# Isaac-McPadden/Farkle_II

Measured on AMD Instinct MI355X. Metric: simulated games/sec (whole node) at k=2, fixed strategy-grid size, higher is better.
Workload: dtype int32; 1 GPU; BASELINE configs[1]: k=2, 64-strategy grid, 10^7 games per GPU per step, root_seed 42, counts-only tallies; k=2, root_seed=42, parallelism=shuffle-range split x1, device=AMD Radeon Graphics, arch=gfx950:sramecc+:xnack-, compute_units=256, clock_mhz=2400

## Files before the change

### farkle_ii_amd/csrc/farkle_hip.hip

```cpp
#include "fk_kernels.h"
#include "fk_shard_writer.h"
#include "fk_perm_wave.h"
#include "fk_row_columns_seats.h"
#include "fk_matchups.h"
#include "fk_game_stats.h"
#include "fk_bootstrap.h"
#include "fk_root_stability.h"

#include <dlfcn.h>
#include <rccl/rccl.h>
#include <unistd.h>

#include <algorithm>
#include <atomic>
#include <chrono>
#include <cmath>
#include <memory>
#include <mutex>
#include <sys/mman.h>
#include <unordered_map>
#include <thread>
#include <cstdarg>
#include <cstdio>
#include <cstring>
// ... 51 lines not shown
    int32_t hint_state = 0, pipeline = 1;
    hipDeviceProp_t prop{};
    std::string err;
    fk_timing timing{};
    std::string play_instance;
    hipEvent_t ev[8] = {nullptr, nullptr, nullptr, nullptr, nullptr, nullptr, nullptr, nullptr};
    int32_t *err_host = nullptr;
    hipEvent_t main_idle = nullptr;
    struct PendingTimer {
        float *acc;
        hipEvent_t a, b;
    };
    std::vector<PendingTimer> pending;
    DevBuf strat, recs, rec0, tally, rows, ov, seatlist, coords, inv, slow, score_lut, discard_lut, block_out, stats, ratios, digest,
        dbg[6];
    std::vector<uint2> strat_host;
    int32_t longest_first = 1;
    int32_t blocks_per_cu = 0;
    int32_t max_waves = 6;
    int32_t lean = -1;
    int32_t gs = -1;
    int32_t uniform_flags_opt = -1;
    uint32_t table_flags = 0;
    uint32_t table_mixed_flags = 0xff00u;
    int64_t chunk_bytes = (int64_t)48 << 30;
    int32_t workspace_percent = 80;
    int64_t chunk_limit = 0;
    int64_t last_budget = 0;
    bool oom = false;
    std::vector<void *> hog;
    int32_t oom_replays = 0;
    int32_t batch_threshold = 0;
    int32_t use_lds_tally = -1;
    int32_t block = 0;
    int32_t hc = -1;
    int32_t hc_waves = 5;
    int32_t hc_block = 256;
    int32_t hc_tables = 1;
    int32_t hc_inc_regs = 1;
    int32_t hc_cl = -1;
    DevBuf lds_tables;
    DevBuf cold;
    int32_t clock_stamps = 0;
    DevBuf clk;
    int clk_grid = 0;
    DevBuf lag_v, lag_out, lag_lags, lag_edge, lag_tmp;
    DevBuf m_ids, m_dig, m_seat, m_rnd;
    DevBuf mr[36];
    uint64_t matchup_sort_mask = ~0ull;
    DevBuf g_rec, g_out;
    int64_t game_stats_window = 0;
    const GameStatsReq *gstats = nullptr;
    DevBuf rootb[4];
    DevBuf boot[8];
    int64_t bootstrap_block = 0;
    bool ran_hc = false;
    int32_t perm_split = -1;
    int32_t columns_by_seat = -1;
    int32_t perm_draw_wave = -1;
    void *comm = nullptr;
    int comm_rank = 0, comm_world = 1;
    bool comm_async = false;
    bool comm_lost = false;
    bool comm_timeout_set = false;
    int32_t comm_timeout_ms = 120000;
    DevBuf comm_buf;
// ... 146 lines not shown
    for (int64_t i = 0; i < S; ++i)
        if (s[i].consider_dice && (s[i].require_both || !s[i].consider_score))
            patience[(size_t)i] = s[i].dice_threshold < 1 ? 3 : s[i].dice_threshold == 1 ? 2 : s[i].dice_threshold == 2 ? 1 : 0;
    rc = ensure(c, c->slow, patience.size());
    if (rc) return rc;
    HIPCHK(c, hipMemcpyAsync(c->slow.p, patience.data(), patience.size(), hipMemcpyHostToDevice, c->stream));
    HIPCHK(c, hipStreamSynchronize(c->stream));
    c->strat_host.swap(packed);
    return FK_OK;
}

SeedPool seed_prefix(uint32_t purpose, uint64_t root_seed, uint64_t k) {
    SeedPool p;
    ss_begin(p, 2u , purpose, (uint32_t)root_seed, (uint32_t)(root_seed >> 32));
    ss_absorb64(p, k);
    return p;
}

struct LaunchPlan {
    int block = 0, grid = 0, cus = 1;
    mutable int launched_grid = 0;
    mutable const char *instance = nullptr;
    size_t lds = 0;
    bool lds_tally = false;
    bool lean = false;
    bool gs = false;
    bool blk = false;
    bool hc = false;
    bool hc_lt = false;
    int hc_ki = 0;
    bool hc_cl = false;
    int wpe = 4;
    uint32_t mixed_flags = 0xff00u;
};

constexpr size_t LDS_LIMIT = 160 * 1024;

size_t play_lds_bytes(int32_t k, int block, bool lean, bool gs, bool lds_tally, int32_t S, bool blocks_mode = false) {
    const size_t per_lane = (size_t)(lean ? LEAN_DW : NF) * 4 * (size_t)(gs ? 1 : k) + (blocks_mode ? 4 : 0);
    return per_lane * (size_t)block + (lds_tally ? (size_t)S * LT_COLS * 8 : 0);
}

LaunchPlan plan_play(const fk_ctx *c, int32_t k, int64_t S, bool single_batch, int32_t target_score, bool blocks_mode = false) {
    LaunchPlan best;
    const bool lean_ok = ceil_div50(target_score) <= LEAN_MAX_TARGET50;
    if (blocks_mode) {
        if (!lean_ok) return best;
        best.block = 768;
        best.lean = true;
        best.blk = true;
        best.wpe = 6;
        best.lds = play_lds_bytes(2, 768, true, false, false, 0, true);
        const int per_cu = c->blocks_per_cu > 0 ? std::min(2, c->blocks_per_cu) : 2;
        best.grid = c->prop.multiProcessorCount * per_cu;
        best.cus = c->prop.multiProcessorCount;
        return best;
    }
    const bool want_tally = single_batch && !blocks_mode && (c->use_lds_tally != 0) && S <= 4096;
    int best_lanes = -1;
    const bool gs_wanted = c->gs == 1;
    for (int gs = 0; gs <= 1; ++gs) {
        if (gs != (gs_wanted ? 1 : 0) && best_lanes >= 0) continue;
        for (int lean = 0; lean <= 1; ++lean) {
            if (gs && !lean) continue;
            if (lean && !lean_ok) continue;
            if (!gs && c->lean >= 0 && lean != c->lean) continue;
// ... 184 lines not shown
hipError_t launch_play_hc(const LaunchPlan &p, const PlayArgs &a, hipStream_t s) {
    if (p.hc_cl) {
        if (p.block == 320 && a.k <= 4u) return launch_play_hc_t<320, false, 0, 6, false, true, 4>(p, a, s);
        return hipErrorInvalidValue;
    }
    if (p.hc_ki == 3) {
        if (p.block != 768) return hipErrorInvalidValue;
        if (a.k <= 10u) return launch_play_hc_t<768, true, 10, 3, false, false, 10>(p, a, s);
        return launch_play_hc_t<768, true, 12, 3, false, false, 12>(p, a, s);
    }
    if (p.hc_ki == 2) {
        if (a.k == 5u && p.block == 256) return launch_play_hc_t<256, true, 5, 4, false, false, 6>(p, a, s);
        if (a.k == 6u && p.block == 512) return launch_play_hc_t<512, true, 6, 4, false, false, 6>(p, a, s);
        if (a.k == 7u && p.block == 1024) return launch_play_hc_t<1024, true, 7, 4, false>(p, a, s);
        return hipErrorInvalidValue;
    }
    if (p.hc_ki && p.block == 256 && p.hc_lt) {
        if (a.k == 8u) return launch_play_hc_t<256, true, 8>(p, a, s);
    }
    return hipErrorInvalidValue;
}

hipError_t launch_play(const LaunchPlan &p, const PlayArgs &a, hipStream_t s) {
    if (p.lds > LDS_LIMIT) return hipErrorInvalidValue;
    if (p.hc) return launch_play_hc(p, a, s);
    if (p.blk) return launch_play_t<768, true, 6, false, true, 2>(p, a, s);
    if (p.gs) {
        if (p.block == 768) return launch_play_t<768, true, 6, true>(p, a, s);
        return hipErrorInvalidValue;
    }
    if (p.lean) {
        switch (p.block) {
        case 1024: return launch_play_t<1024, true>(p, a, s);
        case 768: return a.k == 2u ? launch_play_t<768, true, 6, false, false, 2>(p, a, s) : launch_play_t<768, true, 6>(p, a, s);
        case 512: return launch_play_t<512, true>(p, a, s);
        case 256: return launch_play_t<256, true>(p, a, s);
        case 128: return launch_play_t<128, true>(p, a, s);
        default: return launch_play_t<64, true>(p, a, s);
        }
    }
    switch (p.block) {
    case 1024: return launch_play_t<1024, false>(p, a, s);
    case 512: return launch_play_t<512, false>(p, a, s);
    case 256: return launch_play_t<256, false>(p, a, s);
    case 128: return launch_play_t<128, false>(p, a, s);
    default: return launch_play_t<64, false>(p, a, s);
    }
}

enum TimerSlot : int { SLOT_PERM = 0, SLOT_SEED = 2, SLOT_PLAY = 4, SLOT_CALL = 6 };

struct Timer {
    fk_ctx *c;
    float *acc;
    hipEvent_t a, b;
    Timer(fk_ctx *ctx, float *dst, int slot) : c(ctx), acc(dst), a(ctx->ev[slot]), b(ctx->ev[slot + 1]) {
        (void)hipEventRecord(a, c->stream);
    }
    void stop() {
        (void)hipEventRecord(b, c->stream);
        c->pending.push_back({acc, a, b});
    }
};

hipError_t collect_timers(fk_ctx *c) {
    hipError_t first = hipSuccess;
    for (const auto &t : c->pending) {
// ... 137 lines not shown
                           sa.blocks ? sa.game_row : nullptr, static_cast<uint32_t *>(cs.classes.p));
    hipLaunchKernelGGL(fk_seed_kernel, dim3((sa.n_games + SEED_BLOCK - 1u) / SEED_BLOCK), dim3(SEED_BLOCK), 0, st, sa);
    if (timed) (void)hipEventRecord(cs.ev[3], st);
    HIPCHK(c, hipGetLastError());
    return FK_OK;
}

size_t game_workspace_bytes(int32_t k, bool full_state, bool recs, bool rows) {
    return (size_t)k * ((full_state ? STATE_DW * 4 : 18) + 16) + 8 + (recs ? REC_DW * 4 + 4 : 0) +
           (rows ? sizeof(fk_row_hdr) + sizeof(fk_seat) * (size_t)k : 0);
}

int launch_play_stage(fk_ctx *c, const SeedArgs &sa, PlayArgs &pa, const LaunchPlan &plan, bool want_state, bool want_rec0, bool want_recs) {
    ChunkSet &cs = CSET(c);
    int rc;
    if (want_rec0) {
        rc = ensure(c, c->rec0, (size_t)sa.n_games * 4);
        if (rc) return rc;
    }
    if (want_recs) {
        rc = ensure(c, c->recs, (size_t)sa.n_games * REC_DW * 4);
        if (rc) return rc;
    }
    pa.sched = sa.sched;
    pa.seat_idx = sa.seat_idx;
    pa.state = sa.state;
    pa.state_dw = sa.state_dw;
    pa.inc = sa.inc;
    pa.rec0 = want_rec0 ? static_cast<uint32_t *>(c->rec0.p) : nullptr;
    pa.recs = want_recs ? static_cast<uint32_t *>(c->recs.p) : nullptr;
    pa.gs_out = (want_state && !plan.gs) ? 1u : 0u;
    pa.ticket = static_cast<uint32_t *>(cs.misc.p);
    pa.err = reinterpret_cast<int32_t *>(static_cast<uint8_t *>(cs.misc.p) + 16);
    const int auto_thr = sa.k >= 11 ? 16 : sa.k >= 9 ? 12 : 8;
    pa.batch_threshold = (uint32_t)std::max(1, std::min(64, c->batch_threshold > 0 ? c->batch_threshold : auto_thr));
    pa.use_lds_tally = plan.lds_tally ? 1u : 0u;
    pa.clk = nullptr;
    c->clk_grid = 0;
    if (c->clock_stamps) {
        const size_t bytes = (size_t)std::max(plan.grid, 1) * 4 * sizeof(unsigned long long);
        rc = ensure(c, c->clk, bytes);
        if (rc) return rc;
        HIPCHK(c, hipMemsetAsync(c->clk.p, 0, bytes, c->stream));
        pa.clk = static_cast<unsigned long long *>(c->clk.p);
    }
    {
        Timer t(c, &c->timing.play_ms, SLOT_PLAY);
        LaunchPlan lp = plan;
        lp.mixed_flags = (c->uniform_flags_opt != 0) ? c->table_mixed_flags : 0xff00u;
        pa.uflags = c->table_flags;
        hipError_t e = launch_play(lp, pa, c->stream);
        t.stop();
        HIPCHK(c, e);
        c->play_instance = lp.instance ? lp.instance : "";
        c->timing.play_grid = lp.launched_grid;
        c->timing.play_mixed_flags = lp.mixed_flags == MIXED_NONE ? (int32_t)MIXED_NONE
                                     : (lp.mixed_flags & ~MIXED_RB_FAV) == 0u ? (int32_t)MIXED_RB_FAV : (int32_t)MIXED_ALL;
        if (pa.clk) c->clk_grid = lp.launched_grid;
    }
    c->timing.play_launches += 1;
    c->timing.play_block = plan.block;
    c->timing.play_lds_bytes = (int32_t)plan.lds;
    c->timing.games += sa.n_games;
    return FK_OK;
}

int finish_timers(fk_ctx *c) {
    HIPCHK(c, collect_timers(c));
    if (c->clk_grid > 0) {
        std::vector<unsigned long long> h((size_t)c->clk_grid * 4);
        HIPCHK(c, hipMemcpy(h.data(), c->clk.p, h.size() * sizeof(unsigned long long), hipMemcpyDeviceToHost));
        std::vector<double> mhz, ends;
        unsigned long long first = ~0ull;
        for (int b = 0; b < c->clk_grid; ++b) {
            const unsigned long long t0 = h[(size_t)b * 4], r0 = h[(size_t)b * 4 + 1], t1 = h[(size_t)b * 4 + 2], r1 = h[(size_t)b * 4 + 3];
            if (r1 > r0 && t1 > t0) {
                mhz.push_back(100.0 * (double)(t1 - t0) / (double)(r1 - r0));
                ends.push_back((double)r1);
                first = r0 < first ? r0 : first;
            }
        }
// ... 493 lines not shown
    if (free_now) *free_now = (int64_t)free_b;
    if (total) *total = (int64_t)total_b;
    return FK_OK;
}

static int32_t effective_comm_timeout_ms(const fk_ctx *c);

int fk_get_option(fk_ctx *c, const char *name, int64_t *value) {
    if (!c || !name || !value) return FK_ERR_ARG;
    const std::string n(name);
    if (n == "chunk_bytes") *value = c->chunk_bytes;
    else if (n == "workspace_percent") *value = c->workspace_percent;
    else if (n == "last_budget") *value = c->last_budget;
    else if (n == "oom_replays") *value = c->oom_replays;
    else if (n == "comm_timeout_ms") *value = effective_comm_timeout_ms(c);
    else if (n == "rows_chunk_games") *value = c->rows_chunk_games;
    else if (n == "rows_async") *value = c->rows_async;
    else if (n == "rows_event") *value = c->last_rows_event;
    else return fail(c, FK_ERR_ARG, "fk_get_option: unknown option %s", name);
    return FK_OK;
}

int fk_set_option(fk_ctx *c, const char *name, int64_t value) {
    if (!c || !name) return FK_ERR_ARG;
    std::string n(name);
    if (n == "chunk_bytes") c->chunk_bytes = std::max<int64_t>(value, 1 << 20);
    else if (n == "workspace_percent") c->workspace_percent = (int32_t)std::min<int64_t>(std::max<int64_t>(value, 1), 100000);
    else if (n == "comm_timeout_ms") {
        c->comm_timeout_ms = (int32_t)std::min<int64_t>(std::max<int64_t>(value, 0), 86400000);
        c->comm_timeout_set = true;
    }
    else if (n == "batch_threshold") c->batch_threshold = (int32_t)value;
    else if (n == "use_lds_tally") c->use_lds_tally = (int32_t)value;
    else if (n == "longest_first") c->longest_first = (int32_t)value;
    else if (n == "blocks_per_cu") c->blocks_per_cu = (int32_t)value;
    else if (n == "max_waves") c->max_waves = (int32_t)std::min<int64_t>(std::max<int64_t>(value, 1), 8);
    else if (n == "lean") c->lean = (int32_t)value;
    else if (n == "state_store") c->gs = (int32_t)value;
    else if (n == "rows_chunk_games") c->rows_chunk_games = std::max<int64_t>(value, 1);
    else if (n == "rows_async") c->rows_async = value != 0;
    else if (n == "resident_tally") {
        c->resident = value != 0;
        c->acc_n = 0;
    } else if (n == "hot_cold") {
        if (value != -1 && value != 0) return fail(c, FK_ERR_ARG, "hot_cold is -1 (auto: four and more seats) or 0 (never)");
        c->hc = (int32_t)value;
    }
    else if (n == "clock_stamps") c->clock_stamps = value != 0;
    else if (n == "perm_split") c->perm_split = (int32_t)value;
    else if (n == "perm_draw_wave") c->perm_draw_wave = (int32_t)value;
    else if (n == "columns_by_seat") c->columns_by_seat = (int32_t)value;
    else if (n == "pipeline") c->pipeline = (int32_t)value;
    else if (n == "uniform_flags") c->uniform_flags_opt = (int32_t)value;
    else if (n == "matchup_sort_key_mask") c->matchup_sort_mask = (uint64_t)value;
    else if (n == "game_stats_window") c->game_stats_window = std::max<int64_t>(value, 0);
    else if (n == "bootstrap_block") c->bootstrap_block = std::max<int64_t>(value, 0);
    else if (n == "block") {
        if (value != 0 && value != 64 && value != 128 && value != 256 && value != 512 && value != 768 && value != 1024)
            return fail(c, FK_ERR_ARG, "block must be 0, 64, 128, 256, 512, 768 (lean records only) or 1024");
        c->block = (int32_t)value;
    } else return fail(c, FK_ERR_ARG, "unknown option %s", name);
    return FK_OK;
}

int fk_tournament_run(fk_ctx *c, const fk_strategy *strategies, int32_t S, int32_t k, uint64_t root_seed,
                      uint64_t shuffle_begin, uint64_t shuffle_end, uint32_t shuffles_per_batch, int32_t target_score,
// ... 1807 lines not shown
```

### farkle_ii_amd/csrc/fk_kernels.h

```cpp
#pragma once

#include "../../include/farkle_hip.h"
#include "fk_device.h"

#include <hip/hip_runtime.h>

using namespace fk;

namespace {

constexpr uint32_t HC_AFTER_6_WORDS = ss_hc(24);
constexpr uint32_t HC_AFTER_12_WORDS = ss_hc(48);
constexpr uint32_t HC_AFTER_14_WORDS = ss_hc(56);

enum : uint32_t { MODE_PERM = 0, MODE_LIST = 1, MODE_BLOCKS = 2 };

enum : uint32_t {
    F_LO0 = 0, F_LO1, F_HI0, F_HI1, F_INC_LO0, F_INC_LO1, F_INC_HI0, F_INC_HI1,
    F_BUF, F_SCORE, F_CA, F_CB, F_CC, F_CD, F_CE, F_SPX, F_SPY, NF
};
constexpr uint32_t CE_HAS_SCORED = 1u << 16, CE_HAS_BUF = 1u << 17;
constexpr uint32_t CE_IDX_SHIFT = 18;
constexpr uint32_t LEAN_DW = 10;
constexpr int32_t LEAN_MAX_TARGET50 = 64000;
// ... 66 lines not shown
    uint32_t n_games, gps, n_sh, k, S;
    int32_t target50;
    int32_t beat50;
    uint32_t max_rounds;
    uint32_t batch_threshold;
    uint32_t use_lds_tally;
    uint32_t uflags;
    uint4 *cold;
    const uint8_t *lds_tables;
    unsigned long long *clk;
};

__device__ inline void clock_stamp(unsigned long long *clk, uint32_t which) {
    if (!clk) return;
    unsigned long long *slot = clk + (size_t)blockIdx.x * 4u + 2u * which;
    if (which == 0u) {
        if (threadIdx.x == 0) {
            slot[0] = __builtin_amdgcn_s_memtime();
            slot[1] = __builtin_amdgcn_s_memrealtime();
        }
    } else if ((threadIdx.x & 63u) == 0u) {
        atomicMax(slot, (unsigned long long)__builtin_amdgcn_s_memtime());
        atomicMax(slot + 1, (unsigned long long)__builtin_amdgcn_s_memrealtime());
    }
}

__device__ inline uint32_t lane_id() { return threadIdx.x & 63u; }

__device__ inline uint32_t mbcnt(uint64_t mask) {
    return __builtin_amdgcn_mbcnt_hi((uint32_t)(mask >> 32), __builtin_amdgcn_mbcnt_lo((uint32_t)mask, 0u));
}

__device__ inline Strat unpack_strat(uint2 v) { return Strat{(int32_t)v.x, v.y}; }

__device__ inline uint32_t perm_at(const uint16_t *perm, uint32_t S, uint32_t slots, uint32_t sh, uint32_t e) {
    const uint32_t b = sh / slots, l = sh - b * slots;
    return perm[((size_t)b * S + e) * slots + l];
}

constexpr int PERM_BLOCK = 512, PERM_WAVES = PERM_BLOCK / 64;

__global__ __launch_bounds__(PERM_BLOCK) void fk_perm_kernel(SeedPool prefix, uint64_t shuffle0, uint32_t n_sh, uint32_t S,
                                                             uint32_t slots, uint16_t *perm_T) {
    extern __shared__ uint16_t perm_lds[];
    const uint32_t per_wave = (slots + PERM_WAVES - 1u) / PERM_WAVES;
    const uint32_t wave = threadIdx.x >> 6, lane = threadIdx.x & 63u;
    const uint32_t slot = wave * per_wave + lane;
    const uint32_t sh = blockIdx.x * slots + slot;
    const bool valid = lane < per_wave && slot < slots && sh < n_sh;
    uint16_t *a = perm_lds + (size_t)(valid ? slot : 0u) * S;
    if (valid) {
        for (uint32_t e = 0; e < S; ++e) a[e] = (uint16_t)e;
    }
    Rng r{};
    if (valid) {
        SeedPool p = prefix;
        p.hc = HC_AFTER_6_WORDS;
        ss_absorb64(p, shuffle0 + sh);
#pragma unroll
        for (int w = 0; w < 5; ++w) ss_absorb64(p, 0);
        uint32_t g8[8];
        ss_generate<8>(p, g8);
        pcg_seed(r, g8);
    }
    uint32_t i = valid ? S - 1u : 0u;
    auto consume = [&](uint32_t w) {
// ... 474 lines not shown
}

template <int BLOCK, bool LEAN, int WPE, uint32_t MIXED, bool GS, bool BLK = false, int KC = 0>
__global__ __launch_bounds__(BLOCK) __attribute__((amdgpu_waves_per_eu(WPE))) void fk_play_kernel(PlayArgs a) {
    static_assert(!GS || LEAN, "state-store instances stage the lean record");
    static_assert(!BLK || (LEAN && !GS), "block-index instances use lean LDS records");
    extern __shared__ __attribute__((aligned(16))) uint32_t lds[];
    const uint32_t tid = threadIdx.x;
    const uint32_t K = KC ? (uint32_t)KC : a.k;
    constexpr uint32_t NFIELDS = LEAN ? LEAN_DW : (uint32_t)NF;
    unsigned long long *tl = reinterpret_cast<unsigned long long *>(lds + NFIELDS * (GS ? 1u : K) * BLOCK);
    uint32_t *lane_block = lds + NFIELDS * (GS ? 1u : K) * BLOCK + tid;
    clock_stamp(a.clk, 0u);

    if (a.use_lds_tally) {
        for (uint32_t i = tid; i < a.S * LT_COLS; i += BLOCK) tl[i] = 0ull;
        __syncthreads();
    }

    enum : uint32_t { ST_FRESH = 0, ST_ACTIVE = 1, ST_ENDED = 2, ST_DONE = 3 };
    uint32_t st = ST_FRESH;
    uint32_t pool_next = 0, pool_end = 0, exhausted = 0;

    uint32_t game_id = 0, seat = 0, rounds = 0, max_rounds = 0, trigger = 0, seed_slot = 0;
    uint32_t final_round = 0, safety = 0;
    int32_t score_to_beat = 0;
    uint32_t dice = 6, rolls_this_turn = 0;
    int32_t turn_score = 0;
    uint32_t own_turns = 0;
    uint64_t own_inc_lo = 0, own_inc_hi = 0;
    int32_t own_thr = 0;
    uint32_t own_bits = 0;
    constexpr bool PK2 = (KC == 2) && LEAN && !GS;
    uint2 pk_seat0 = make_uint2(0u, 0u), pk_seat1 = make_uint2(0u, 0u);

    const uint32_t lane_base = tid * NFIELDS;
    constexpr uint32_t SEAT_STRIDE = (uint32_t)BLOCK * NFIELDS;
    auto L = [&](uint32_t field, uint32_t s) __attribute__((always_inline)) -> uint32_t & {
        const uint32_t f = !LEAN ? field : (field > F_SCORE) ? field - 5u : (field > F_INC_HI1) ? field - 4u : field;
        if (GS) return lds[lane_base + f];
        return lds[__umul24(s, SEAT_STRIDE) + lane_base + f];
    };
    auto G = [&](uint32_t s) __attribute__((always_inline)) -> uint32_t * {
        return a.state + ((size_t)seed_slot * K + s) * a.state_dw;
    };

    auto strategy_index = [&](uint32_t id, uint32_t s) -> uint32_t {
        if (a.mode == MODE_PERM) {
            const uint32_t sh = id / a.gps, g = id - sh * a.gps;
            return perm_at(a.perm_T, a.S, a.perm_slots, sh, g * K + s);
        }
        if (a.mode == MODE_LIST) return (uint32_t)a.seat_strategy[(size_t)id * K + s];
        return 2u * a.game_block[id] + s;
    };

    auto seat_strategy = [&](uint32_t s) -> uint32_t {
        if (GS) return G(s)[R_IDX];
        if (BLK) return 2u * *lane_block + s;
        if (LEAN) return L(F_CE, s) >> CE_IDX_SHIFT;
        return strategy_index(game_id, s);
    };
    auto seat_score = [&](uint32_t s) -> int32_t {
        return (int32_t)(GS ? G(s)[R_SCORE] : LEAN ? (L(F_CE, s) & 0xffffu) : L(F_SCORE, s));
    };
    auto seat_counter = [&](uint32_t s, uint32_t field) -> uint32_t {
        return GS ? G(s)[R_CA + (field - F_CA)] : L(field, s);
// ... 13 lines not shown
            r[1] = make_uint2(q0.z, q0.w);
            r[2] = make_uint2(q1.x, q1.z);
            r[3] = make_uint2((q1.w & 0xffffu) | (q2.z << 16), q2.x);
            r[4] = make_uint2(q2.y, (q1.y & 0xffffu) | (q2.z & (CE_HAS_SCORED | CE_HAS_BUF)));
            own_turns = (q1.w >> 16) + 1u;
            idx = q2.w;
        } else if (!PK2) {
            if (BLK) idx = 2u * *lane_block + s;
            else if (LEAN) idx = L(F_CE, s) >> CE_IDX_SHIFT;
        }
        if (LEAN) {
            const uint4 inc = a.inc[(size_t)seed_slot * K + s];
            const uint2 pk = PK2 ? (s ? pk_seat1 : pk_seat0) : a.strat[idx];
            own_inc_lo = (uint64_t)inc.x | ((uint64_t)inc.y << 32);
            own_inc_hi = (uint64_t)inc.z | ((uint64_t)inc.w << 32);
            own_thr = (int32_t)pk.x;
            own_bits = pk.y;
        } else {
            own_inc_lo = (uint64_t)L(F_INC_LO0, s) | ((uint64_t)L(F_INC_LO1, s) << 32);
            own_inc_hi = (uint64_t)L(F_INC_HI0, s) | ((uint64_t)L(F_INC_HI1, s) << 32);
            own_thr = (int32_t)L(F_SPX, s);
            own_bits = L(F_SPY, s);
        }
        dice = 6;
        turn_score = 0;
        rolls_this_turn = 0;
    };

    auto raise = [&](int32_t code) {
        if (atomicCAS(&a.err[0], 0, code) == 0) a.err[1] = (int32_t)game_id;
        st = ST_DONE;
    };

    auto finish_game = [&]() {
        const bool completed = (safety == 0u);
        uint32_t w = 0;
        int32_t best = seat_score(0);
        for (uint32_t s = 1; s < K; ++s) {
            const int32_t sc = seat_score(s);
            if (sc > best) {
                best = sc;
                w = s;
            }
        }
        if (!GS && a.gs_out) {
            for (uint32_t s = 0; s < K; ++s) {
                uint4 *g = reinterpret_cast<uint4 *>(G(s));
                g[0] = make_uint4(L(F_LO0, s), L(F_LO1, s), L(F_HI0, s), L(F_HI1, s));
                g[1] = make_uint4(L(F_BUF, s), (uint32_t)seat_score(s), L(F_CA, s), (L(F_CB, s) & 0xffffu) | (seat_turns(s) << 16));
                g[2] = make_uint4(L(F_CC, s), L(F_CD, s), seat_hot_dice(s) | (L(F_CE, s) & (CE_HAS_SCORED | CE_HAS_BUF)),
                                  seat_strategy(s));
            }
        }
        if (a.use_lds_tally) {
            if (!completed || a.mode != MODE_PERM) {
                for (uint32_t s = 0; s < K; ++s) atomicAdd(&tl[seat_strategy(s) * LT_COLS + (completed ? 1u : 2u)], 1ull);
            }
        }
        if (!(a.use_lds_tally && completed) && !a.rec0) return;
        uint32_t widx = 0, wa = 0, wb = 0, wc = 0, wd = 0, we = 0;
        if (completed) {
            widx = seat_strategy(w);
            wa = seat_counter(w, F_CA), wb = seat_counter(w, F_CB), wc = seat_counter(w, F_CC), wd = seat_counter(w, F_CD),
            we = seat_hot_dice(w);
        } else if (a.mode == MODE_BLOCKS) {
            widx = seat_strategy(0);
        }
        if (a.use_lds_tally && completed) {
            const unsigned long long m[10] = {(unsigned long long)(uint32_t)best * 50u, rounds, wa >> 16, wa & 0xffffu,
                                              (wb & 0xffffu) * 50u, wc & 0xffffu, wc >> 16, wd & 0xffffu, wd >> 16, we};
            unsigned long long *t = tl + widx * LT_COLS;
            atomicAdd(&t[0], 1ull);
#pragma unroll
            for (int j = 0; j < 10; ++j) {
                if (m[j]) {
                    atomicAdd(&t[3 + j], m[j]);
                    atomicAdd(&t[13 + j], m[j] * m[j]);
                }
            }
        }
        if (a.rec0) {
            const uint32_t d0 = widx | (completed ? (w << 24) : REC_SAFETY);
            a.rec0[game_id] = d0;
            if (a.recs) {
                uint4 *r = reinterpret_cast<uint4 *>(a.recs + (size_t)game_id * REC_DW);
                r[0] = make_uint4(d0, completed ? (uint32_t)best * 50u : 0u, rounds | (wa & 0xffff0000u),
// ... 43 lines not shown
                    L(F_SPX, s) = pk.x;
                    L(F_SPY, s) = pk.y;
                }
                L(F_BUF, s) = 0u;
                if (!LEAN) L(F_SCORE, s) = 0u;
                L(F_CA, s) = 0u;
                L(F_CB, s) = 0u;
                L(F_CC, s) = 0u;
                L(F_CD, s) = 0u;
                L(F_CE, s) = (LEAN && !BLK) ? (idx << CE_IDX_SHIFT) : 0u;
                if (PK2) {
                    const uint2 pk = a.strat[BLK ? 2u * a.game_block[id] + s : idx];
                    if (s == 0u) pk_seat0 = pk;
                    else pk_seat1 = pk;
                }
            }
        }
        seat = 0;
        trigger = 0;
        final_round = 0;
        safety = 0;
        score_to_beat = a.beat50;
        if (max_rounds == 0u) {
            rounds = 0;
            safety = 1;
            st = ST_ENDED;
        } else {
            rounds = 1;
            begin_turn(0);
            st = ST_ACTIVE;
        }
    };

    auto advance = [&](int32_t score) __attribute__((always_inline)) {
        const bool fr = final_round != 0u;
        const bool trig = !fr & (score >= a.target50);
        const bool normal = !fr & !trig;
        const uint32_t n1 = seat + 1u;
        const bool wrap = n1 == K;
        const bool last = normal & wrap & (rounds >= max_rounds);
        uint32_t next_fr = n1 + ((n1 == trigger) ? 1u : 0u);
        uint32_t next_tr = (seat == 0u) ? 1u : 0u, next_nm = wrap ? 0u : n1;
        asm volatile("" : "+v"(next_fr), "+v"(next_tr), "+v"(next_nm));
        const uint32_t next = fr ? next_fr : trig ? next_tr : next_nm;
        rounds += (normal & wrap & !last) ? 1u : 0u;
        safety = last ? 1u : safety;
        score_to_beat = trig ? score : (fr & (score > score_to_beat)) ? score : score_to_beat;
        trigger = trig ? seat : trigger;
        final_round = (fr | trig) ? 1u : 0u;
        const bool ended = last | ((fr | trig) & (next >= K));
        if (ended) {
            st = ST_ENDED;
        } else {
            seat = next;
            begin_turn(next);
        }
    };

    auto advance2 = [&](bool over, int32_t score) __attribute__((always_inline)) {
        const bool fr = final_round != 0u;
        const bool trig = over & !fr & (score >= a.target50);
        const bool close = over & !fr & !trig & (seat != 0u);
        const bool last = close & (rounds >= max_rounds);
        const bool ended = last | (over & fr);
        rounds += (close & !last) ? 1u : 0u;
        safety = last ? 1u : safety;
        score_to_beat = trig ? score : score_to_beat;
        trigger = trig ? seat : trigger;
        final_round = (fr | trig) ? 1u : 0u;
        const bool sw = over & !ended;
        st = ended ? (uint32_t)ST_ENDED : st;
        seat ^= sw ? 1u : 0u;
        if (sw) {
            const uint4 inc = a.inc[(size_t)seed_slot * 2u + seat];
            own_inc_lo = (uint64_t)inc.x | ((uint64_t)inc.y << 32);
            own_inc_hi = (uint64_t)inc.z | ((uint64_t)inc.w << 32);
        }
        own_thr = (int32_t)(seat ? pk_seat1.x : pk_seat0.x);
        own_bits = seat ? pk_seat1.y : pk_seat0.y;
        dice = sw ? 6u : dice;
        turn_score = sw ? 0 : turn_score;
        rolls_this_turn = sw ? 0u : rolls_this_turn;
    };

    auto roll_step = [&]() __attribute__((always_inline)) {
        const bool roll_limit = rolls_this_turn >= 1000u;
        const uint32_t s = seat;
        uint32_t cA, cB, cC, cD, cE, buf0;
        int32_t score;
        uint64_t lo0, hi0;
        uint2 *const rec = reinterpret_cast<uint2 *>(&L(F_LO0, s));
        if (LEAN) {
            const uint2 p0 = rec[0], p1 = rec[1], p2 = rec[2], p3 = rec[3], p4 = rec[4];
            lo0 = (uint64_t)p0.x | ((uint64_t)p0.y << 32);
            hi0 = (uint64_t)p1.x | ((uint64_t)p1.y << 32);
            buf0 = p2.x, cA = p2.y, cB = p3.x, cC = p3.y, cD = p4.x, cE = p4.y;
            score = (int32_t)(cE & 0xffffu);
        } else {
            cA = L(F_CA, s), cB = L(F_CB, s), cC = L(F_CC, s), cD = L(F_CD, s), cE = L(F_CE, s);
            score = (int32_t)L(F_SCORE, s);
            lo0 = (uint64_t)L(F_LO0, s) | ((uint64_t)L(F_LO1, s) << 32);
            hi0 = (uint64_t)L(F_HI0, s) | ((uint64_t)L(F_HI1, s) << 32);
            buf0 = L(F_BUF, s);
        }
        Rng rng{hi0, lo0, own_inc_hi, own_inc_lo, buf0, (cE & CE_HAS_BUF) ? 1u : 0u};
        const uint32_t n = dice;
        bool detour;
        uint32_t key = roll_counts_fast<3>(rng, n, detour);
        if (detour) {
            asm volatile("" ::: "memory");
            rng.lo = (uint64_t)L(F_LO0, s) | ((uint64_t)L(F_LO1, s) << 32);
            rng.hi = (uint64_t)L(F_HI0, s) | ((uint64_t)L(F_HI1, s) << 32);
            rng.buf = L(F_BUF, s);
            rng.has_buf = (cE & CE_HAS_BUF) ? 1u : 0u;
            key = roll_counts_sequential<3>(rng, n, nullptr);
        }
        rolls_this_turn += 1u;
        int32_t dthr = (int32_t)(int8_t)(own_bits & 0xffu);
        asm volatile("" : "+v"(dthr));
        const Strat50 sp{own_thr, (own_bits & (0xffu | MIXED)) | (a.uflags & (0xff00u & ~MIXED)), dthr};
        const Roll50 rr = default_score_lut50(a.score_lut, a.discard_lut, key, (int32_t)n, turn_score, sp);
        const bool farkle = rr.score50 == 0;
        cA += 1u + (farkle ? 0x10000u : 0u);
        cC += (rr.d5 > 0) ? (1u + ((uint32_t)rr.d5 << 16)) : 0u;
        cD += (rr.d1 > 0) ? (1u + ((uint32_t)rr.d1 << 16)) : 0u;
        dice = (rr.used == (int32_t)n) ? 6u : (n - (uint32_t)rr.used);
        turn_score = farkle ? 0 : (turn_score + rr.score50);
        const bool hot = !farkle & sp.has(SF_AUTO_HOT) & (dice == 6u);
        if (LEAN) cB += hot ? 0x10000u : 0u;
        else cE += hot ? 1u : 0u;
        const bool keep = should_continue50(sp, turn_score, (int32_t)dice, (cE & CE_HAS_SCORED) != 0u, final_round != 0u,
                                            score_to_beat, score);
        const bool over = farkle | (!hot & !keep);
        const uint32_t ts = over ? (uint32_t)turn_score : 0u;
        cE |= (ts >= 10u) ? CE_HAS_SCORED : 0u;
        const uint32_t banked = (cE & CE_HAS_SCORED) ? ts : 0u;
        score += (int32_t)banked;
        if (LEAN) cE += banked;
        cB = (banked > (cB & 0xffffu)) ? ((cB & 0xffff0000u) | banked) : cB;
        const bool overflow = (turn_score > 1310) | ((cA & 0xffffu) > 64000u) | ((cC >> 16) > 63000u) | ((cD >> 16) > 63000u);
        if (roll_limit | overflow) {
            raise(roll_limit ? FK_ERR_ROLL_LIMIT : FK_ERR_COUNTER_OVERFLOW);
            return;
        }
        cE = (cE & ~CE_HAS_BUF) | (rng.has_buf ? CE_HAS_BUF : 0u);
        if (GS) {
// ... 4 lines not shown
                uint32_t *g2 = reinterpret_cast<uint32_t *>(g + 2);
                g2[0] = cC;
                g2[1] = cD;
                g2[2] = (cB >> 16) | (cE & (CE_HAS_SCORED | CE_HAS_BUF));
                advance(score);
                return;
            }
        }
        if (LEAN) {
            rec[0] = make_uint2((uint32_t)rng.lo, (uint32_t)(rng.lo >> 32));
            rec[1] = make_uint2((uint32_t)rng.hi, (uint32_t)(rng.hi >> 32));
            rec[2] = make_uint2(rng.buf, cA);
            rec[3] = make_uint2(cB, cC);
            rec[4] = make_uint2(cD, cE);
        } else {
            L(F_LO0, s) = (uint32_t)rng.lo;
            L(F_LO1, s) = (uint32_t)(rng.lo >> 32);
            L(F_HI0, s) = (uint32_t)rng.hi;
            L(F_HI1, s) = (uint32_t)(rng.hi >> 32);
            L(F_BUF, s) = rng.buf;
            L(F_SCORE, s) = (uint32_t)score;
            L(F_CA, s) = cA;
            L(F_CB, s) = cB;
            L(F_CC, s) = cC;
            L(F_CD, s) = cD;
            L(F_CE, s) = cE;
        }
        if (PK2) advance2(over, score);
        else if (!GS && over) advance(score);
    };

    auto handover = [&](uint64_t waiting) {
        const bool mine = (st == ST_FRESH || st == ST_ENDED);
        if (st == ST_ENDED) finish_game();
        const uint32_t n = (uint32_t)__popcll(waiting);
        const uint32_t avail = pool_end - pool_next;
        uint32_t new_base = 0, new_avail = 0;
        if (avail < n && !exhausted) {
            const uint32_t first = (uint32_t)__builtin_amdgcn_readfirstlane(__ffsll((long long)waiting) - 1);
            uint32_t base = 0;
            if (mine && lane_id() == first) base = atomicAdd(a.ticket, TICKET_CHUNK);
            base = (uint32_t)__builtin_amdgcn_readlane((int)base, (int)first);
            if (base >= a.n_games) {
                exhausted = 1;
            } else {
                new_base = base;
                new_avail = min(TICKET_CHUNK, a.n_games - base);
                if (new_avail < TICKET_CHUNK) exhausted = 1;
            }
        }
        if (mine) {
            const uint32_t rank = mbcnt(waiting);
            uint32_t ticket = 0xffffffffu;
            if (rank < avail) ticket = pool_next + rank;
            else if (rank - avail < new_avail) ticket = new_base + (rank - avail);
            if (ticket != 0xffffffffu) init_game(a.sched ? a.sched[ticket] : ticket, ticket);
            else st = ST_DONE;
        }
        if (n <= avail) {
            pool_next += n;
        } else {
            const uint32_t used_new = min(n - avail, new_avail);
            pool_next = new_base + used_new;
            pool_end = new_base + new_avail;
        }
    };

    auto handover_due = [&](uint64_t waiting, uint64_t active) -> bool {
        return waiting && (!active || (uint32_t)__popcll(waiting) >= a.batch_threshold || exhausted);
    };
    while (true) {
        uint64_t waiting = __ballot(st == ST_FRESH || st == ST_ENDED);
        uint64_t active = __ballot(st == ST_ACTIVE);
        if (!(waiting | active)) break;
        if (handover_due(waiting, active)) {
            handover(waiting);
            continue;
        }
        do {
            if (st == ST_ACTIVE) roll_step();
            waiting = __ballot(st == ST_ENDED);
            active = __ballot(st == ST_ACTIVE);
        } while (active && !handover_due(waiting, active));
    }

    if (a.use_lds_tally) {
        __syncthreads();
        for (uint32_t i = tid; i < a.S * LT_COLS; i += BLOCK) {
            const unsigned long long v = tl[i];
            if (v == 0ull) continue;
            const uint32_t idx = i / LT_COLS, c = i - idx * LT_COLS;
            if (c == LT_COLS - 1u) continue;
            const uint32_t col = (c == 0u) ? 0u : (c == 1u) ? 2u : (c == 2u) ? 3u : (c < 13u) ? (c + 1u) : (c + 2u);
            atomicAdd(&a.tally[(size_t)idx * FK_TALLY_COLS + col], v);
        }
    }
    clock_stamp(a.clk, 1u);
}

#include "fk_play_hc.h"

constexpr uint32_t LAG_WIN_BIT = 0x8000u;

__global__ __launch_bounds__(256) void fk_lag_values_kernel(const uint32_t *recs, const uint16_t *perm_T, uint32_t perm_slots, uint32_t S,
                                                            uint32_t k, uint32_t gps, uint32_t n_games, uint16_t *V) {
    const size_t t = (size_t)blockIdx.x * blockDim.x + threadIdx.x;
    if (t >= (size_t)n_games * k) return;
    const uint32_t id = (uint32_t)(t / k), seat = (uint32_t)(t - (size_t)id * k);
    const uint32_t sh = id / gps, g = id - sh * gps;
    const uint4 q0 = *reinterpret_cast<const uint4 *>(recs + (size_t)id * REC_DW);
// ... 566 lines not shown
```

Measured before the change: 1.110 billion games/s.

## Add specialized k=2 lean handover path with 32-bit offsets and inlined init/finish

For the k=2 lean non-blocks kernel, adds specialized finish_game2/init_game2 routines that use 32-bit byte offsets, packed per-seat loads and direct LDS record addressing. The handover loop now re-checks state after a handover and falls straight into rolling instead of looping back. A host-side check falls back to the generic kernel whenever offsets could overflow 32 bits, and a wide_offsets option can force that fallback. The aim is to cut address arithmetic, register use and loop overhead in the per-game handover, at the cost of a duplicated code path that must stay consistent with the generic one.

```diff
diff --git a/farkle_ii_amd/csrc/farkle_hip.hip b/farkle_ii_amd/csrc/farkle_hip.hip
--- a/farkle_ii_amd/csrc/farkle_hip.hip
+++ b/farkle_ii_amd/csrc/farkle_hip.hip
@@ -107,6 +107,7 @@
     int32_t oom_replays = 0;
     int32_t batch_threshold = 0;
     int32_t use_lds_tally = -1;
+    int32_t wide_offsets = -1;
     int32_t block = 0;
     int32_t hc = -1;
     int32_t hc_waves = 5;
@@ -319,6 +320,7 @@
     bool hc_cl = false;
     int wpe = 4;
     uint32_t mixed_flags = 0xff00u;
+    bool wide = false;
 };
 
 constexpr size_t LDS_LIMIT = 160 * 1024;
@@ -569,7 +571,7 @@
     if (p.lean) {
         switch (p.block) {
         case 1024: return launch_play_t<1024, true>(p, a, s);
-        case 768: return a.k == 2u ? launch_play_t<768, true, 6, false, false, 2>(p, a, s) : launch_play_t<768, true, 6>(p, a, s);
+        case 768: return (a.k == 2u && !p.wide) ? launch_play_t<768, true, 6, false, false, 2>(p, a, s) : launch_play_t<768, true, 6>(p, a, s);
         case 512: return launch_play_t<512, true>(p, a, s);
         case 256: return launch_play_t<256, true>(p, a, s);
         case 128: return launch_play_t<128, true>(p, a, s);
@@ -773,6 +775,8 @@
     pa.gs_out = (want_state && !plan.gs) ? 1u : 0u;
     pa.ticket = static_cast<uint32_t *>(cs.misc.p);
     pa.err = reinterpret_cast<int32_t *>(static_cast<uint8_t *>(cs.misc.p) + 16);
+    const uint64_t per_game = std::max<uint64_t>((uint64_t)sa.k * std::max<uint64_t>(sa.state_dw * 4u, 16u), REC_DW * 4u);
+    const bool wide = c->wide_offsets > 0 || (std::max((uint64_t)sa.n_games * per_game, (uint64_t)pa.S * 8u) >> 32) != 0;
     const int auto_thr = sa.k >= 11 ? 16 : sa.k >= 9 ? 12 : 8;
     pa.batch_threshold = (uint32_t)std::max(1, std::min(64, c->batch_threshold > 0 ? c->batch_threshold : auto_thr));
     pa.use_lds_tally = plan.lds_tally ? 1u : 0u;
@@ -788,6 +792,7 @@
     {
         Timer t(c, &c->timing.play_ms, SLOT_PLAY);
         LaunchPlan lp = plan;
+        lp.wide = wide;
         lp.mixed_flags = (c->uniform_flags_opt != 0) ? c->table_mixed_flags : 0xff00u;
         pa.uflags = c->table_flags;
         hipError_t e = launch_play(lp, pa, c->stream);
@@ -1347,6 +1352,7 @@
     }
     else if (n == "batch_threshold") c->batch_threshold = (int32_t)value;
     else if (n == "use_lds_tally") c->use_lds_tally = (int32_t)value;
+    else if (n == "wide_offsets") c->wide_offsets = (int32_t)value;
     else if (n == "longest_first") c->longest_first = (int32_t)value;
     else if (n == "blocks_per_cu") c->blocks_per_cu = (int32_t)value;
     else if (n == "max_waves") c->max_waves = (int32_t)std::min<int64_t>(std::max<int64_t>(value, 1), 8);
diff --git a/farkle_ii_amd/csrc/fk_kernels.h b/farkle_ii_amd/csrc/fk_kernels.h
--- a/farkle_ii_amd/csrc/fk_kernels.h
+++ b/farkle_ii_amd/csrc/fk_kernels.h
@@ -122,6 +122,15 @@
 }
 
 __device__ inline Strat unpack_strat(uint2 v) { return Strat{(int32_t)v.x, v.y}; }
+
+template <typename T, typename OFF>
+__device__ inline T ld_at(const void *base, OFF byte_off) {
+    return *reinterpret_cast<const T *>(static_cast<const char *>(base) + byte_off);
+}
+template <typename T, typename OFF>
+__device__ inline void st_at(void *base, OFF byte_off, T v) {
+    *reinterpret_cast<T *>(static_cast<char *>(base) + byte_off) = v;
+}
 
 __device__ inline uint32_t perm_at(const uint16_t *perm, uint32_t S, uint32_t slots, uint32_t sh, uint32_t e) {
     const uint32_t b = sh / slots, l = sh - b * slots;
@@ -662,6 +671,7 @@
     int32_t own_thr = 0;
     uint32_t own_bits = 0;
     constexpr bool PK2 = (KC == 2) && LEAN && !GS;
+    constexpr bool LHO = PK2 && !BLK;
     uint2 pk_seat0 = make_uint2(0u, 0u), pk_seat1 = make_uint2(0u, 0u);
 
     const uint32_t lane_base = tid * NFIELDS;
@@ -741,6 +751,16 @@
         st = ST_DONE;
     };
 
+    auto flush_records = [&]() {
+        for (uint32_t s = 0; s < K; ++s) {
+            uint4 *g = reinterpret_cast<uint4 *>(G(s));
+            g[0] = make_uint4(L(F_LO0, s), L(F_LO1, s), L(F_HI0, s), L(F_HI1, s));
+            g[1] = make_uint4(L(F_BUF, s), (uint32_t)seat_score(s), L(F_CA, s), (L(F_CB, s) & 0xffffu) | (seat_turns(s) << 16));
+            g[2] = make_uint4(L(F_CC, s), L(F_CD, s), seat_hot_dice(s) | (L(F_CE, s) & (CE_HAS_SCORED | CE_HAS_BUF)),
+                              seat_strategy(s));
+        }
+    };
+
     auto finish_game = [&]() {
         const bool completed = (safety == 0u);
         uint32_t w = 0;
@@ -752,15 +772,7 @@
                 w = s;
             }
         }
-        if (!GS && a.gs_out) {
-            for (uint32_t s = 0; s < K; ++s) {
-                uint4 *g = reinterpret_cast<uint4 *>(G(s));
-                g[0] = make_uint4(L(F_LO0, s), L(F_LO1, s), L(F_HI0, s), L(F_HI1, s));
-                g[1] = make_uint4(L(F_BUF, s), (uint32_t)seat_score(s), L(F_CA, s), (L(F_CB, s) & 0xffffu) | (seat_turns(s) << 16));
-                g[2] = make_uint4(L(F_CC, s), L(F_CD, s), seat_hot_dice(s) | (L(F_CE, s) & (CE_HAS_SCORED | CE_HAS_BUF)),
-                                  seat_strategy(s));
-            }
-        }
+        if (!GS && a.gs_out) flush_records();
         if (a.use_lds_tally) {
             if (!completed || a.mode != MODE_PERM) {
                 for (uint32_t s = 0; s < K; ++s) atomicAdd(&tl[seat_strategy(s) * LT_COLS + (completed ? 1u : 2u)], 1ull);
@@ -870,6 +882,128 @@
         }
     };
 
+    using OFF = uint32_t;
+    auto finish_game2 = [&]() __attribute__((always_inline)) {
+        const bool completed = (safety == 0u);
+        const uint32_t ce0 = L(F_CE, 0), ce1 = L(F_CE, 1);
+        const uint32_t sc0 = ce0 & 0xffffu, sc1 = ce1 & 0xffffu;
+        const uint32_t w = (sc1 > sc0) ? 1u : 0u;
+        const uint32_t best = w ? sc1 : sc0;
+        const uint32_t idx0 = ce0 >> CE_IDX_SHIFT, idx1 = ce1 >> CE_IDX_SHIFT;
+        if (a.gs_out) flush_records();
+        if (a.use_lds_tally && (!completed || a.mode != MODE_PERM)) {
+            const uint32_t col = completed ? 1u : 2u;
+            atomicAdd(&tl[idx0 * LT_COLS + col], 1ull);
+            atomicAdd(&tl[idx1 * LT_COLS + col], 1ull);
+        }
+        const bool tally_w = a.use_lds_tally && completed;
+        if (!tally_w && !a.rec0) return;
+        const uint2 *wr = reinterpret_cast<const uint2 *>(&L(F_LO0, w));
+        const uint2 p2 = wr[2], p3 = wr[3], p4 = wr[4];
+        const uint32_t wa = p2.y, wb = p3.x, wc = p3.y, wd = p4.x, we = p3.x >> 16;
+        const uint32_t widx = w ? idx1 : idx0;
+        if (tally_w) {
+            unsigned long long *t = tl + widx * LT_COLS;
+            auto add = [&](uint32_t j, uint32_t v) __attribute__((always_inline)) {
+                atomicAdd(&t[3u + j], (unsigned long long)v);
+                atomicAdd(&t[13u + j], (unsigned long long)v * v);
+            };
+            atomicAdd(&t[0], 1ull);
+            add(0, best * 50u);
+            add(1, rounds);
+            add(2, wa >> 16);
+            add(3, wa & 0xffffu);
+            add(4, (wb & 0xffffu) * 50u);
+            if (wc | wd) {
+                add(5, wc & 0xffffu);
+                add(6, wc >> 16);
+                add(7, wd & 0xffffu);
+                add(8, wd >> 16);
+            }
+            if (we) add(9, we);
+        }
+        if (a.rec0) {
+            const uint32_t ridx = completed ? widx : (a.mode == MODE_BLOCKS) ? idx0 : 0u;
+            const uint32_t d0 = ridx | (completed ? (w << 24) : REC_SAFETY);
+            st_at<uint32_t>(a.rec0, (OFF)game_id * 4u, d0);
+            if (a.recs) {
+                const uint32_t ra = completed ? wa : 0u, rb = completed ? (wb & 0xffffu) * 50u : 0u;
+                const OFF ro = (OFF)game_id * (REC_DW * 4u);
+                st_at<uint4>(a.recs, ro, make_uint4(d0, completed ? best * 50u : 0u, rounds | (ra & 0xffff0000u), (ra & 0xffffu) | (rb << 16)));
+                st_at<uint4>(a.recs, ro + 16u, make_uint4(completed ? wc : 0u, completed ? wd : 0u, completed ? we : 0u, 0u));
+            }
+        }
+    };
+
+    auto init_game2 = [&](uint32_t ticket) __attribute__((always_inline)) {
+        uint32_t id = ticket;
+        if (a.sched) id = ld_at<uint32_t>(a.sched, (OFF)ticket * 4u);
+        uint32_t mr = a.max_rounds;
+        if (a.n_ov) {
+            uint32_t lo = 0, hi = a.n_ov;
+            while (lo < hi) {
+                const uint32_t mid = (lo + hi) >> 1;
+                if (a.ov[mid].game < id) lo = mid + 1u;
+                else hi = mid;
+            }
+            if (lo < a.n_ov && a.ov[lo].game == id) mr = a.ov[lo].max_rounds;
+        }
+        uint32_t slot = ticket;
+        if (!a.sched) {
+            slot = id;
+            if (a.mode == MODE_PERM) {
+                const uint32_t sh = id / a.gps, g = id - sh * a.gps;
+                slot = g * a.n_sh + sh;
+            }
+        }
+        const uint32_t seat_bytes = a.state_dw * 4u;
+        const OFF sb = (OFF)slot * (2u * seat_bytes);
+        const char *state1 = reinterpret_cast<const char *>(a.state) + seat_bytes;
+        const uint4 s0 = ld_at<uint4>(a.state, sb), s1 = ld_at<uint4>(state1, sb);
+        const uint4 inc = ld_at<uint4>(a.inc, (OFF)slot * 32u);
+        uint32_t idx0, idx1;
+        if (a.state_dw == STATE_DW) {
+            idx0 = ld_at<uint32_t>(a.state, sb + R_IDX * 4u), idx1 = ld_at<uint32_t>(state1, sb + R_IDX * 4u);
+        } else if (a.seat_idx) {
+            const uint32_t two = ld_at<uint32_t>(a.seat_idx, (OFF)slot * 4u);
+            idx0 = two & 0xffffu, idx1 = two >> 16;
+        } else {
+            idx0 = strategy_index(id, 0u), idx1 = strategy_index(id, 1u);
+        }
+        const uint2 pk0 = ld_at<uint2>(a.strat, (OFF)idx0 * 8u), pk1 = ld_at<uint2>(a.strat, (OFF)idx1 * 8u);
+        uint2 *r0 = reinterpret_cast<uint2 *>(&L(F_LO0, 0u)), *r1 = reinterpret_cast<uint2 *>(&L(F_LO0, 1u));
+        r0[0] = make_uint2(s0.x, s0.y);
+        r0[1] = make_uint2(s0.z, s0.w);
+        r0[2] = make_uint2(0u, 0u);
+        r0[3] = make_uint2(0u, 0u);
+        r0[4] = make_uint2(0u, idx0 << CE_IDX_SHIFT);
+        r1[0] = make_uint2(s1.x, s1.y);
+        r1[1] = make_uint2(s1.z, s1.w);
+        r1[2] = make_uint2(0u, 0u);
+        r1[3] = make_uint2(0u, 0u);
+        r1[4] = make_uint2(0u, idx1 << CE_IDX_SHIFT);
+        const bool none = (mr == 0u);
+        game_id = id;
+        max_rounds = mr;
+        seed_slot = slot;
+        pk_seat0 = pk0;
+        pk_seat1 = pk1;
+        seat = 0;
+        trigger = 0;
+        final_round = 0;
+        score_to_beat = a.beat50;
+        rounds = none ? 0u : 1u;
+        safety = none ? 1u : 0u;
+        st = none ? (uint32_t)ST_ENDED : (uint32_t)ST_ACTIVE;
+        own_inc_lo = (uint64_t)inc.x | ((uint64_t)inc.y << 32);
+        own_inc_hi = (uint64_t)inc.z | ((uint64_t)inc.w << 32);
+        own_thr = (int32_t)pk0.x;
+        own_bits = pk0.y;
+        dice = 6;
+        turn_score = 0;
+        rolls_this_turn = 0;
+    };
+
     auto advance = [&](int32_t score) __attribute__((always_inline)) {
         const bool fr = final_round != 0u;
         const bool trig = !fr & (score >= a.target50);
@@ -927,7 +1061,12 @@
         uint32_t cA, cB, cC, cD, cE, buf0;
         int32_t score;
         uint64_t lo0, hi0;
-        uint2 *const rec = reinterpret_cast<uint2 *>(&L(F_LO0, s));
+        uint2 *rec = reinterpret_cast<uint2 *>(&L(F_LO0, s));
+        if (LHO) {
+            uint32_t rbase = __umul24(s, SEAT_STRIDE) + lane_base;
+            asm volatile("" : "+v"(rbase));
+            rec = reinterpret_cast<uint2 *>(lds + rbase);
+        }
         if (LEAN) {
             const uint2 p0 = rec[0], p1 = rec[1], p2 = rec[2], p3 = rec[3], p4 = rec[4];
             lo0 = (uint64_t)p0.x | ((uint64_t)p0.y << 32);
@@ -947,9 +1086,16 @@
         uint32_t key = roll_counts_fast<3>(rng, n, detour);
         if (detour) {
             asm volatile("" ::: "memory");
-            rng.lo = (uint64_t)L(F_LO0, s) | ((uint64_t)L(F_LO1, s) << 32);
-            rng.hi = (uint64_t)L(F_HI0, s) | ((uint64_t)L(F_HI1, s) << 32);
-            rng.buf = L(F_BUF, s);
+            if (LHO) {
+                const uint2 q0 = rec[0], q1 = rec[1];
+                rng.lo = (uint64_t)q0.x | ((uint64_t)q0.y << 32);
+                rng.hi = (uint64_t)q1.x | ((uint64_t)q1.y << 32);
+                rng.buf = rec[2].x;
+            } else {
+                rng.lo = (uint64_t)L(F_LO0, s) | ((uint64_t)L(F_LO1, s) << 32);
+                rng.hi = (uint64_t)L(F_HI0, s) | ((uint64_t)L(F_HI1, s) << 32);
+                rng.buf = L(F_BUF, s);
+            }
             rng.has_buf = (cE & CE_HAS_BUF) ? 1u : 0u;
             key = roll_counts_sequential<3>(rng, n, nullptr);
         }
@@ -1020,7 +1166,10 @@
 
     auto handover = [&](uint64_t waiting) {
         const bool mine = (st == ST_FRESH || st == ST_ENDED);
-        if (st == ST_ENDED) finish_game();
+        if (st == ST_ENDED) {
+            if (LHO) finish_game2();
+            else finish_game();
+        }
         const uint32_t n = (uint32_t)__popcll(waiting);
         const uint32_t avail = pool_end - pool_next;
         uint32_t new_base = 0, new_avail = 0;
@@ -1037,7 +1186,13 @@
                 if (new_avail < TICKET_CHUNK) exhausted = 1;
             }
         }
-        if (mine) {
+        if (LHO) {
+            const uint32_t rank = mbcnt(waiting);
+            const bool valid = rank < avail || rank - avail < new_avail;
+            const uint32_t ticket = (rank < avail) ? pool_next + rank : new_base + (rank - avail);
+            st = (mine && !valid) ? (uint32_t)ST_DONE : st;
+            if (mine && valid) init_game2(ticket);
+        } else if (mine) {
             const uint32_t rank = mbcnt(waiting);
             uint32_t ticket = 0xffffffffu;
             if (rank < avail) ticket = pool_next + rank;
@@ -1063,7 +1218,10 @@
         if (!(waiting | active)) break;
         if (handover_due(waiting, active)) {
             handover(waiting);
-            continue;
+            if (!LHO) continue;
+            waiting = __ballot(st == ST_FRESH || st == ST_ENDED);
+            active = __ballot(st == ST_ACTIVE);
+            if (!active || handover_due(waiting, active)) continue;
         }
         do {
             if (st == ST_ACTIVE) roll_step();
```

After: 1.143 billion games/s, median of 6. +3.0%, better.
